# cts198859/deeprl_network

Measured on NVIDIA H100. Metric: agent-env-steps/sec CACC Catch-up NeurComm A2C, higher is better.
Workload: dtype f32

## Files before the change

### deeprl_network_b200/csrc/tc_wgrad.cu

```cuda
#include "bwd_common.cuh"
#include "tc_row.cuh"

extern long long* g_nmarl_prof;

namespace {
using namespace tcrow;

enum { J_GATE0 = 0, J_GATE1, J_ENC_X, J_ENC_M0, J_ENC_M1, J_COUNT };
constexpr int WG_LANES = 128, WG_HALF = 64;
constexpr int WG_A_THREADS = WG_LANES, WG_THREADS = WG_A_THREADS + 2 * 128;
constexpr uint32_t WG_A_TILE = WG_LANES * 128, WG_A_SLOT = 2 * WG_A_TILE;
constexpr uint32_t WG_RING = 224 * 1024;
constexpr int WG_MAX_BARS = 32;
constexpr size_t WG_SMEM = 1024 + WG_RING + WG_MAX_BARS * 8;
static_assert(WG_SMEM <= 232448, "wgrad rings exceed the 227 KB of dynamic shared memory");
static_assert(WG_HALF == ROWS, "each MMA warpgroup covers the 64 rows of one wgmma");
constexpr int WG_REGS_A = 120, WG_REGS_MMA = 192;
static_assert(WG_A_THREADS * WG_REGS_A + 256 * WG_REGS_MMA <= WG_THREADS * 168, "setmaxnreg split exceeds the CTA's registers");
constexpr int SEG_KB = 20;

__device__ __forceinline__ void wg_depths(int N, int& S, int& A) {
  S = N >= 256 ? 2 : (N >= 192 ? 3 : (N >= 128 ? 4 : 6));
  A = (int)((WG_RING - (uint32_t)S * 256u * (uint32_t)N) / WG_A_SLOT);
  if (A > 4) A = 4;
}

struct RingPos {
  int idx = 0; uint32_t ph = 0;
  __device__ __forceinline__ void next(int n) { if (++idx == n) { idx = 0; ph ^= 1u; } }
};

struct TcWgK {
  int B, T, splits, ndp;
  const float* sv_sh; const float* sv_xin; const float* dzT; const float* dpT;
  const float* h_seq; const float* done_pre;
  float* ws;
  long long ws_off[J_COUNT];
  int jobs[J_COUNT]; int n_jobs;
  int* err;
  long long* prof;
};

struct JobDesc {
  const float* A; int F_A, a_feat0, ka_cnt, ones;
  int p_feat0, p_cnt;
  const float* BT; int tile_rows, n_row0, N;
};

__device__ __forceinline__ JobDesc job_desc(const nmarl_model& m, const TcWgK& k, int kind, int i) {
  const nmarl_agent& ag = m.agent[i];
  JobDesc d;
  d.p_feat0 = 0; d.p_cnt = 0;
  const int SD = m.s_dim, LDI = m.kx_pad + m.kp_pad + m.km_pad;
  const int Km = (m.variant == NMARL_IC3) ? NH : ag.n_nbr * NH;
  if (kind == J_GATE0 || kind == J_GATE1) {
    const int mt = kind - J_GATE0;
    d.A = k.sv_sh; d.F_A = SD + NH; d.a_feat0 = 128 * mt; d.ka_cnt = max(0, min(128, SD + NH - 128 * mt)); d.ones = 0;
    d.BT = k.dzT; d.tile_rows = 256; d.n_row0 = 0; d.N = 256;
  } else if (kind == J_ENC_X) {
    d.A = k.sv_xin; d.F_A = LDI; d.a_feat0 = 0; d.ka_cnt = ag.x_nsrc * ag.x_w; d.ones = 1;
    if (m.variant == NMARL_NC) { d.p_feat0 = m.kx_pad; d.p_cnt = ag.n_nbr * m.n_a; }
    d.BT = k.dpT; d.tile_rows = k.ndp; d.n_row0 = 0; d.N = k.ndp;
  } else {
    const int mt = kind - J_ENC_M0;
    d.A = k.sv_xin; d.F_A = LDI; d.a_feat0 = m.kx_pad + m.kp_pad + 128 * mt; d.ka_cnt = max(0, min(128, Km - 128 * mt)); d.ones = 0;
    d.BT = k.dpT; d.tile_rows = k.ndp; d.n_row0 = (m.variant == NMARL_NC) ? 128 : 64; d.N = 64;
  }
  return d;
}

template <bool RAW>
__global__ void __launch_bounds__(WG_THREADS, 1) tc_wgrad_kernel(const __grid_constant__ nmarl_model m,
                                                                 const __grid_constant__ TcWgK k) {
  extern __shared__ uint8_t smem_raw[];
  uint8_t* smem = reinterpret_cast<uint8_t*>((reinterpret_cast<uintptr_t>(smem_raw) + 1023) & ~uintptr_t(1023));

  const int sp = blockIdx.x, jslot = blockIdx.y, i = blockIdx.z;
  const int kind = k.jobs[jslot];
  const JobDesc d = job_desc(m, k, kind, i);
  const int lanes = d.ka_cnt > 0 ? d.ka_cnt + d.ones + d.p_cnt : 0;
  const int nact = (lanes + WG_HALF - 1) / WG_HALF;
  if (nact == 0) return;
  int S, AS;
  wg_depths(d.N, S, AS);
  uint8_t* bst = smem;
  uint8_t* ast = smem + (size_t)S * 256 * d.N;
  uint64_t* bars = reinterpret_cast<uint64_t*>(smem + WG_RING);
  uint64_t *b_full = bars, *b_split = b_full + S, *b_empty = b_split + S, *a_full = b_empty + S, *a_empty = a_full + AS;

  const int N_agents = m.n_agent;
  const int tid = threadIdx.x, warp = tid >> 5;
  const int bpt = k.B / 32;
  const int kb_total = k.T * bpt;
  const int per = (kb_total + k.splits - 1) / k.splits;
  const int kb0 = sp * per, kb1 = min(kb_total, kb0 + per);
  const int nkb = (d.ka_cnt > 0) ? max(0, kb1 - kb0) : 0;
  float* wsj = k.ws + k.ws_off[jslot] + ((size_t)sp * N_agents + i) * 128 * d.N;

  if (tid == 0) {
    for (int s = 0; s < S; ++s) { tc::mbar_init(&b_full[s], 1); tc::mbar_init(&b_split[s], WG_A_THREADS); tc::mbar_init(&b_empty[s], 4 * nact); }
    for (int s = 0; s < AS; ++s) { tc::mbar_init(&a_full[s], WG_A_THREADS); tc::mbar_init(&a_empty[s], 4 * nact); }
    tc::fence_barrier_init();
  }
  __syncthreads();
  const uint32_t tile_bytes = (uint32_t)d.N * 128u;

  if (warp < WG_A_THREADS / 32) {
    asm volatile("setmaxnreg.dec.sync.aligned.u32 %0;" ::"n"(WG_REGS_A));
    const int row = tid;
    const bool on = row < WG_HALF * nact;
    const int ka = row;
    const bool one = d.ones && ka == d.ka_cnt;
    const bool is_p = ka > d.ka_cnt && ka <= d.ka_cnt + d.p_cnt;
    const bool real = on && (ka < d.ka_cnt || is_p);
    const int feat = is_p ? d.p_feat0 + (ka - d.ka_cnt - 1) : d.a_feat0 + ka;
    int hs_agent = -1, hs_unit = 0;
    bool hs_mask = false;
    if (k.h_seq != nullptr && real && !is_p) {
      if ((kind == J_GATE0 || kind == J_GATE1) && feat >= m.s_dim) { hs_agent = i; hs_unit = feat - m.s_dim; hs_mask = true; }
      else if ((kind == J_ENC_M0 || kind == J_ENC_M1) && m.variant == NMARL_NC) {
        const int fm = feat - (m.kx_pad + m.kp_pad);
        hs_agent = m.agent[i].nbr[fm / NH]; hs_unit = fm % NH;
      }
    }
    auto load_x = [&](int q, float (&x)[32]) {
      const int kb = kb0 + q, t = kb / bpt, rb = kb - t * bpt;
      if (hs_agent >= 0) {
        const float* src = k.h_seq + (((size_t)t * N_agents + hs_agent) * NH + hs_unit) * k.B + rb * 32;
#pragma unroll
        for (int p = 0; p < 8; ++p) {
          const float4 v = __ldg(reinterpret_cast<const float4*>(src + 4 * p));
          x[4 * p] = v.x; x[4 * p + 1] = v.y; x[4 * p + 2] = v.z; x[4 * p + 3] = v.w;
        }
        if (hs_mask) {
          const float* dn = k.done_pre + (size_t)t * k.B + rb * 32;
#pragma unroll
          for (int p = 0; p < 8; ++p) {
            const float4 v = __ldg(reinterpret_cast<const float4*>(dn + 4 * p));
            x[4 * p] *= 1.0f - v.x; x[4 * p + 1] *= 1.0f - v.y; x[4 * p + 2] *= 1.0f - v.z; x[4 * p + 3] *= 1.0f - v.w;
          }
        }
      } else if (real) {
        const float* src = d.A + (((size_t)t * N_agents + i) * d.F_A + feat) * k.B + rb * 32;
#pragma unroll
        for (int p = 0; p < 8; ++p) {
          const float4 v = __ldcs(reinterpret_cast<const float4*>(src + 4 * p));
          x[4 * p] = v.x; x[4 * p + 1] = v.y; x[4 * p + 2] = v.z; x[4 * p + 3] = v.w;
        }
      } else {
#pragma unroll
        for (int j = 0; j < 32; ++j) x[j] = one ? 1.0f : 0.0f;
      }
    };
    float xa[32], xb[32];
    RingPos as, bs;
    auto emit_a = [&](int q, float (&x)[32]) {
      tc::mbar_wait(&a_empty[as.idx], as.ph ^ 1, k.err, 11);
      if (on) {
        uint8_t* hi = ast + (size_t)as.idx * WG_A_SLOT;
#pragma unroll
        for (int c = 0; c < 4; ++c) {
          float x8[8];
#pragma unroll
          for (int j = 0; j < 8; ++j) x8[j] = x[8 * c + j];
          tc::st_hilo8(hi, hi + WG_A_TILE, (uint32_t)row, (uint32_t)(8 * c), x8);
        }
        tc::fence_proxy_async();
      }
      tc::mbar_arrive(&a_full[as.idx]);
      as.next(AS);
      if (q + 2 < nkb) load_x(q + 2, x);
      if constexpr (RAW) {
        tc::mbar_wait(&b_full[bs.idx], bs.ph, k.err, 31);
        float4* bhi = reinterpret_cast<float4*>(bst + (size_t)bs.idx * 2 * tile_bytes);
        float4* blo = reinterpret_cast<float4*>(bst + (size_t)bs.idx * 2 * tile_bytes + tile_bytes);
        for (uint32_t e = (uint32_t)tid; e < tile_bytes / 16; e += WG_A_THREADS) {
          const float4 v = bhi[e];
          float4 h, lo4;
          tc::split_tf32(v.x, h.x, lo4.x); tc::split_tf32(v.y, h.y, lo4.y);
          tc::split_tf32(v.z, h.z, lo4.z); tc::split_tf32(v.w, h.w, lo4.w);
          bhi[e] = h;
          blo[e] = lo4;
        }
        tc::fence_proxy_async();
        tc::mbar_arrive(&b_split[bs.idx]);
        bs.next(S);
      }
    };
    if (nkb > 0) load_x(0, xa);
    if (nkb > 1) load_x(1, xb);
    for (int q = 0; q < nkb; q += 2) {
      emit_a(q, xa);
      if (q + 1 < nkb) emit_a(q + 1, xb);
    }
  } else {
    const int g = warp / 4 - 1;
    if (g >= nact) return;
    asm volatile("setmaxnreg.inc.sync.aligned.u32 %0;" ::"n"(WG_REGS_MMA));
    const int t = tid - (g + 1) * 128, w = t >> 5, l = t & 31;
    const bool issuer = g == 0 && t == 0;
    float* out = wsj + g * WG_HALF + 16 * w + (l >> 2);
    long long* prof = (issuer && k.prof != nullptr && sp == 0 && i == 0) ? k.prof + (size_t)jslot * 1024 : nullptr;
    if (prof) { prof[0] = clock64(); prof[3] = kind | (d.N << 8); }
    auto fetch = [&](int q, int st) {
      const int kb = kb0 + q;
      const int tt = kb / bpt, rb = kb - tt * bpt;
      const size_t pair = (size_t)(2 * d.tile_rows * 128);
      const size_t off = RAW ? (size_t)tt * N_agents * bpt * pair + ((size_t)i * bpt + rb) * (pair / 2)
                             : (((size_t)tt * N_agents + i) * bpt + rb) * pair;
      const uint8_t* tile = reinterpret_cast<const uint8_t*>(d.BT) + off;
      uint8_t* dst = bst + (size_t)st * 2 * tile_bytes;
      tc::mbar_arrive_expect_tx(&b_full[st], RAW ? tile_bytes : 2 * tile_bytes);
      tc::bulk_g2s(dst, tile + (size_t)d.n_row0 * 128, tile_bytes, &b_full[st]);
      if (!RAW) tc::bulk_g2s(dst + tile_bytes, tile + (size_t)(d.tile_rows + d.n_row0) * 128, tile_bytes, &b_full[st]);
    };
    if (issuer)
      for (int q = 0; q < S && q < nkb; ++q) fetch(q, q);
    float acc[128];
#pragma unroll
    for (int j = 0; j < 128; ++j) acc[j] = 0.f;
    auto drain = [&](bool rmw) {
#pragma unroll
      for (int j = 0; j < 32; ++j) {
        if (8 * j < d.N) {
          const int n = 8 * j + 2 * (l & 3);
#pragma unroll
          for (int e = 0; e < 4; ++e) {
            float* o = out + (size_t)(n + (e & 1)) * 128 + 8 * (e >> 1);
            *o = rmw ? *o + acc[4 * j + e] : acc[4 * j + e];
          }
        }
      }
    };
    RingPos as, bs;
    for (int q = 0; q < nkb; ++q) {
      const bool seg_first = (q % SEG_KB) == 0;
      uint8_t* b = bst + (size_t)bs.idx * 2 * tile_bytes;
      if constexpr (RAW) tc::mbar_wait(&b_split[bs.idx], bs.ph, k.err, 33);
      else tc::mbar_wait(&b_full[bs.idx], bs.ph, k.err, 31);
      if (prof && q < 300) prof[4 + 3 * q] = clock64();
      tc::mbar_wait(&a_full[as.idx], as.ph, k.err, 32);
      if (prof && q < 300) prof[5 + 3 * q] = clock64();
      uint8_t* a = ast + (size_t)as.idx * WG_A_SLOT + g * (WG_A_TILE / 2);
      tc::wgmma_fence();
      tc::wgmma_kblock_3x(d.N, acc, tc::smem_desc_sw128(a), tc::smem_desc_sw128(a + WG_A_TILE), tc::smem_desc_sw128(b),
                          tc::smem_desc_sw128(b + tile_bytes), 4, seg_first);
      tc::wgmma_commit();
      tc::wgmma_wait_all();
      if (prof && q < 300) prof[6 + 3 * q] = clock64();
      if (l == 0) { tc::mbar_arrive(&a_empty[as.idx]); tc::mbar_arrive(&b_empty[bs.idx]); }
      if (issuer && q + S < nkb) {
        tc::mbar_wait(&b_empty[bs.idx], bs.ph, k.err, 34);
        fetch(q + S, bs.idx);
      }
      as.next(AS); bs.next(S);
      if ((q + 1) % SEG_KB == 0 || q + 1 == nkb) drain(q >= SEG_KB);
    }
    if (nkb == 0) drain(false);
    if (prof) { prof[1] = min(nkb, 300); prof[2] = clock64(); }
  }
}

__global__ void __launch_bounds__(256) tc_wgrad_reduce_kernel(const __grid_constant__ nmarl_model m, const __grid_constant__ TcWgK k,
                                                             float* __restrict__ grads) {
  const int jslot = blockIdx.y, i = blockIdx.z, kind = k.jobs[jslot];
  const JobDesc d = job_desc(m, k, kind, i);
  const nmarl_agent& ag = m.agent[i];
  const int lanes = d.ka_cnt + (d.ones ? 1 : 0) + d.p_cnt;
  const int total = 128 * d.N;
  for (int e = blockIdx.x * blockDim.x + threadIdx.x; e < total; e += gridDim.x * blockDim.x) {
    const int ln = e & 127, n = e >> 7;
    if (ln >= lanes) continue;
    float s = 0.f;
    for (int sp = 0; sp < k.splits; ++sp) s += k.ws[k.ws_off[jslot] + (((size_t)sp * m.n_agent + i) * d.N + n) * 128 + ln];
    if (kind == J_GATE0 || kind == J_GATE1) grads[ag.o_wxh + (size_t)(128 * (kind - J_GATE0) + ln) * NG + n] = s;
    else if (kind == J_ENC_X) {
      if (ln < d.ka_cnt) { if (n < NH) grads[ag.o_w_ob + ln * NH + n] = s; }
      else if (ln > d.ka_cnt) { if (n >= NH && n < 2 * NH) grads[ag.o_w_fp + (ln - d.ka_cnt - 1) * NH + n - NH] = s; }
      else if (n < NH) grads[ag.o_b_ob + n] = s;
      else if (m.variant == NMARL_NC && n < 2 * NH) grads[ag.o_b_fp + n - NH] = s;
      else if (ag.o_b_msg >= 0) grads[ag.o_b_msg + n - ((m.variant == NMARL_NC) ? 2 * NH : NH)] = s;
    } else grads[ag.o_w_msg + (size_t)(128 * (kind - J_ENC_M0) + ln) * NH + n] = s;
  }
}

__global__ void __launch_bounds__(256) gate_bias_reduce_kernel(const __grid_constant__ nmarl_model m, const float* __restrict__ part,
                                                              int tiles, int T, float* __restrict__ grads) {
  __shared__ float red[8][32];
  const int c = threadIdx.x & 31, p = threadIdx.x >> 5, col = blockIdx.x * 32 + c, i = blockIdx.y;
  const int n = T * tiles;
  float s = 0.f;
  for (int e = p; e < n; e += 8) {
    const int t = e / tiles, tile = e - t * tiles;
    s += part[(((size_t)t * m.n_agent + i) * tiles + tile) * NG + col];
  }
  red[p][c] = s;
  __syncthreads();
  if (p == 0) {
    float tsum = 0.f;
    for (int w = 0; w < 8; ++w) tsum += red[w][c];
    grads[m.agent[i].o_b + col] = tsum;
  }
}

NMARL_PARAMS_FIT(nmarl_model, TcWgK);
NMARL_PARAMS_FIT(nmarl_model, TcWgK, float*);
NMARL_PARAMS_FIT(nmarl_model, const float*, int, int, float*);

int job_list(const nmarl_model* m, int* jobs) {
  int n = 0;
  jobs[n++] = J_GATE0;
  if (m->s_dim + NH > 128) jobs[n++] = J_GATE1;
  jobs[n++] = J_ENC_X;
  if (m->variant != NMARL_IA2C) {
    jobs[n++] = J_ENC_M0;
    if (m->km_pad > 128) jobs[n++] = J_ENC_M1;
  }
  return n;
}
int job_N(const nmarl_model* m, int kind) {
  if (kind == J_GATE0 || kind == J_GATE1) return 256;
  if (kind == J_ENC_X) return nmarl_tc_ndp(m);
  return 64;
}

}

int nmarl_tc_ndp(const nmarl_model* m) { return m->variant == NMARL_NC ? 192 : (m->variant == NMARL_IA2C ? 64 : 128); }

int nmarl_tc_wgrad_splits(int n_agent) {
  int s = 33;
  while (4 * s * n_agent > 132 * 8 && s > 1) s = (s + 1) / 2;
  return s;
}

int64_t nmarl_tc_wgrad_ws_floats(const nmarl_model* m) {
  int jobs[J_COUNT];
  const int nj = job_list(m, jobs);
  int64_t tot = 0;
  for (int j = 0; j < nj; ++j) tot += (int64_t)nmarl_tc_wgrad_splits(m->n_agent) * m->n_agent * 128 * job_N(m, jobs[j]);
  return tot;
}

int nmarl_tc_launch_wgrads(const nmarl_model* m, int B, int T, const float* sv_sh, const float* sv_xin, const float* dzT,
                           const float* dpT, const float* sv_dz, float* ws, float* grads, int* err, cudaStream_t st,
                           cudaStream_t st_bias, bool raw_tiles, void** ev_wgrad, const float* h_seq, const float* done_pre) {
  TcWgK k{};
  k.B = B; k.T = T; k.splits = nmarl_tc_wgrad_splits(m->n_agent); k.ndp = nmarl_tc_ndp(m);
  k.sv_sh = sv_sh; k.sv_xin = sv_xin; k.dzT = dzT; k.dpT = dpT; k.ws = ws; k.err = err;
  k.h_seq = h_seq; k.done_pre = done_pre; k.prof = g_nmarl_prof;
  k.n_jobs = job_list(m, k.jobs);
  long long off = 0;
  for (int j = 0; j < k.n_jobs; ++j) { k.ws_off[j] = off; off += (long long)k.splits * m->n_agent * 128 * job_N(m, k.jobs[j]); }
  static bool configured = false;
  if (!configured) {
    NMARL_CUDA(cudaFuncSetAttribute(tc_wgrad_kernel<false>, cudaFuncAttributeMaxDynamicSharedMemorySize, (int)WG_SMEM));
    NMARL_CUDA(cudaFuncSetAttribute(tc_wgrad_kernel<true>, cudaFuncAttributeMaxDynamicSharedMemorySize, (int)WG_SMEM));
    configured = true;
  }
  gate_bias_reduce_kernel<<<dim3(NG / 32, m->n_agent), 256, 0, st_bias>>>(*m, sv_dz, B / 32, T, grads);
  NMARL_LAUNCH_CHECK();
  if (ev_wgrad) NMARL_CUDA(cudaEventRecord((cudaEvent_t)ev_wgrad[0], st));
  const dim3 grid(k.splits, k.n_jobs, m->n_agent);
  if (raw_tiles) tc_wgrad_kernel<true><<<grid, WG_THREADS, WG_SMEM, st>>>(*m, k);
  else tc_wgrad_kernel<false><<<grid, WG_THREADS, WG_SMEM, st>>>(*m, k);
  NMARL_LAUNCH_CHECK();
  if (ev_wgrad) NMARL_CUDA(cudaEventRecord((cudaEvent_t)ev_wgrad[1], st));
  NMARL_DBG_SYNC(st, "tc_wgrad_kernel");
  tc_wgrad_reduce_kernel<<<dim3(64, k.n_jobs, m->n_agent), 256, 0, st>>>(*m, k, grads);
  NMARL_LAUNCH_CHECK();
  NMARL_DBG_SYNC(st, "tc_wgrad_reduce");
  return 0;
}
```

Before: 52.82 million.

## Template wgrad MMA loop on N and keep one wgmma group in flight

The MMA warpgroups' main loop moves into a function templated on the tile width N, so the accumulator array and drain loops are sized at compile time instead of a fixed 128-register array with runtime guards. Each k-block's wgmma now waits only on the previous group (wait<1>), overlapping the next block's issue with the current one's completion before releasing ring slots and prefetching. The RAW-mode TF32 hi/lo split loop is also unrolled by four to batch shared-memory loads. In exchange the kernel holds more code per N instantiation, and an unsupported N now reports an error.

```diff
diff --git a/deeprl_network_b200/csrc/tc_wgrad.cu b/deeprl_network_b200/csrc/tc_wgrad.cu
--- a/deeprl_network_b200/csrc/tc_wgrad.cu
+++ b/deeprl_network_b200/csrc/tc_wgrad.cu
@@ -19,10 +19,10 @@
 static_assert(WG_A_THREADS * WG_REGS_A + 256 * WG_REGS_MMA <= WG_THREADS * 168, "setmaxnreg split exceeds the CTA's registers");
 constexpr int SEG_KB = 20;
 
-__device__ __forceinline__ void wg_depths(int N, int& S, int& A) {
-  S = N >= 256 ? 2 : (N >= 192 ? 3 : (N >= 128 ? 4 : 6));
-  A = (int)((WG_RING - (uint32_t)S * 256u * (uint32_t)N) / WG_A_SLOT);
-  if (A > 4) A = 4;
+__host__ __device__ constexpr int wg_stages(int N) { return N >= 256 ? 2 : (N >= 192 ? 3 : (N >= 128 ? 4 : 6)); }
+__host__ __device__ constexpr int wg_slots(int N) {
+  return (WG_RING - (uint32_t)wg_stages(N) * 256u * (uint32_t)N) / WG_A_SLOT >= 4
+             ? 4 : (int)((WG_RING - (uint32_t)wg_stages(N) * 256u * (uint32_t)N) / WG_A_SLOT);
 }
 
 struct RingPos {
@@ -69,6 +69,67 @@
   return d;
 }
 
+struct MmaRing {
+  uint8_t* bst; uint8_t* ast;
+  uint64_t *b_ready; int b_code;
+  uint64_t *b_empty, *a_full, *a_empty;
+  int* err;
+};
+
+template <int N, class Fetch>
+__device__ __forceinline__ void mma_job(const MmaRing& r, int nkb, bool issuer, int l, float* out, long long* prof,
+                                        const Fetch& fetch) {
+  constexpr int S = wg_stages(N), AS = wg_slots(N);
+  constexpr uint32_t TB = (uint32_t)N * 128u;
+  float acc[N / 2];
+#pragma unroll
+  for (int j = 0; j < N / 2; ++j) acc[j] = 0.f;
+  auto drain = [&](bool rmw) {
+#pragma unroll
+    for (int j = 0; j < N / 8; ++j) {
+      const int n = 8 * j + 2 * (l & 3);
+#pragma unroll
+      for (int e = 0; e < 4; ++e) {
+        float* o = out + (size_t)(n + (e & 1)) * 128 + 8 * (e >> 1);
+        *o = rmw ? *o + acc[4 * j + e] : acc[4 * j + e];
+      }
+    }
+  };
+  RingPos as, bs, rb;
+  int ra = 0;
+  auto release = [&](int q) {
+    if (prof && q < 300) prof[6 + 3 * q] = clock64();
+    if (l == 0) { tc::mbar_arrive(&r.a_empty[ra]); tc::mbar_arrive(&r.b_empty[rb.idx]); }
+    if (issuer && q + S < nkb) {
+      tc::mbar_wait(&r.b_empty[rb.idx], rb.ph, r.err, 34);
+      fetch(q + S, rb.idx);
+    }
+    ra = ra + 1 == AS ? 0 : ra + 1;
+    rb.next(S);
+  };
+  for (int q0 = 0; q0 < nkb; q0 += SEG_KB) {
+    const int q1 = min(nkb, q0 + SEG_KB);
+    for (int q = q0; q < q1; ++q) {
+      tc::mbar_wait(&r.b_ready[bs.idx], bs.ph, r.err, r.b_code);
+      if (prof && q < 300) prof[4 + 3 * q] = clock64();
+      tc::mbar_wait(&r.a_full[as.idx], as.ph, r.err, 32);
+      if (prof && q < 300) prof[5 + 3 * q] = clock64();
+      const uint8_t* a = r.ast + (size_t)as.idx * WG_A_SLOT;
+      const uint8_t* b = r.bst + (size_t)bs.idx * 2 * TB;
+      tc::wgmma_fence();
+      tc::wgmma_kblock_3x<N, 4>(acc, tc::smem_desc_sw128(a), tc::smem_desc_sw128(a + WG_A_TILE), tc::smem_desc_sw128(b),
+                                tc::smem_desc_sw128(b + TB), q == q0);
+      tc::wgmma_commit();
+      as.next(AS); bs.next(S);
+      if (q > q0) { tc::wgmma_wait<1>(); release(q - 1); }
+    }
+    tc::wgmma_wait<0>();
+    release(q1 - 1);
+    drain(q0 > 0);
+  }
+  if (nkb == 0) drain(false);
+}
+
 template <bool RAW>
 __global__ void __launch_bounds__(WG_THREADS, 1) tc_wgrad_kernel(const __grid_constant__ nmarl_model m,
                                                                  const __grid_constant__ TcWgK k) {
@@ -81,8 +142,7 @@
   const int lanes = d.ka_cnt > 0 ? d.ka_cnt + d.ones + d.p_cnt : 0;
   const int nact = (lanes + WG_HALF - 1) / WG_HALF;
   if (nact == 0) return;
-  int S, AS;
-  wg_depths(d.N, S, AS);
+  const int S = wg_stages(d.N), AS = wg_slots(d.N);
   uint8_t* bst = smem;
   uint8_t* ast = smem + (size_t)S * 256 * d.N;
   uint64_t* bars = reinterpret_cast<uint64_t*>(smem + WG_RING);
@@ -174,13 +234,18 @@
         tc::mbar_wait(&b_full[bs.idx], bs.ph, k.err, 31);
         float4* bhi = reinterpret_cast<float4*>(bst + (size_t)bs.idx * 2 * tile_bytes);
         float4* blo = reinterpret_cast<float4*>(bst + (size_t)bs.idx * 2 * tile_bytes + tile_bytes);
-        for (uint32_t e = (uint32_t)tid; e < tile_bytes / 16; e += WG_A_THREADS) {
-          const float4 v = bhi[e];
-          float4 h, lo4;
-          tc::split_tf32(v.x, h.x, lo4.x); tc::split_tf32(v.y, h.y, lo4.y);
-          tc::split_tf32(v.z, h.z, lo4.z); tc::split_tf32(v.w, h.w, lo4.w);
-          bhi[e] = h;
-          blo[e] = lo4;
+        for (uint32_t e0 = (uint32_t)tid; e0 < tile_bytes / 16; e0 += 4 * WG_A_THREADS) {
+          float4 v[4];
+#pragma unroll
+          for (int u = 0; u < 4; ++u) v[u] = bhi[e0 + u * WG_A_THREADS];
+#pragma unroll
+          for (int u = 0; u < 4; ++u) {
+            float4 h, lo4;
+            tc::split_tf32(v[u].x, h.x, lo4.x); tc::split_tf32(v[u].y, h.y, lo4.y);
+            tc::split_tf32(v[u].z, h.z, lo4.z); tc::split_tf32(v[u].w, h.w, lo4.w);
+            bhi[e0 + u * WG_A_THREADS] = h;
+            blo[e0 + u * WG_A_THREADS] = lo4;
+          }
         }
         tc::fence_proxy_async();
         tc::mbar_arrive(&b_split[bs.idx]);
@@ -216,47 +281,14 @@
     };
     if (issuer)
       for (int q = 0; q < S && q < nkb; ++q) fetch(q, q);
-    float acc[128];
-#pragma unroll
-    for (int j = 0; j < 128; ++j) acc[j] = 0.f;
-    auto drain = [&](bool rmw) {
-#pragma unroll
-      for (int j = 0; j < 32; ++j) {
-        if (8 * j < d.N) {
-          const int n = 8 * j + 2 * (l & 3);
-#pragma unroll
-          for (int e = 0; e < 4; ++e) {
-            float* o = out + (size_t)(n + (e & 1)) * 128 + 8 * (e >> 1);
-            *o = rmw ? *o + acc[4 * j + e] : acc[4 * j + e];
-          }
-        }
-      }
-    };
-    RingPos as, bs;
-    for (int q = 0; q < nkb; ++q) {
-      const bool seg_first = (q % SEG_KB) == 0;
-      uint8_t* b = bst + (size_t)bs.idx * 2 * tile_bytes;
-      if constexpr (RAW) tc::mbar_wait(&b_split[bs.idx], bs.ph, k.err, 33);
-      else tc::mbar_wait(&b_full[bs.idx], bs.ph, k.err, 31);
-      if (prof && q < 300) prof[4 + 3 * q] = clock64();
-      tc::mbar_wait(&a_full[as.idx], as.ph, k.err, 32);
-      if (prof && q < 300) prof[5 + 3 * q] = clock64();
-      uint8_t* a = ast + (size_t)as.idx * WG_A_SLOT + g * (WG_A_TILE / 2);
-      tc::wgmma_fence();
-      tc::wgmma_kblock_3x(d.N, acc, tc::smem_desc_sw128(a), tc::smem_desc_sw128(a + WG_A_TILE), tc::smem_desc_sw128(b),
-                          tc::smem_desc_sw128(b + tile_bytes), 4, seg_first);
-      tc::wgmma_commit();
-      tc::wgmma_wait_all();
-      if (prof && q < 300) prof[6 + 3 * q] = clock64();
-      if (l == 0) { tc::mbar_arrive(&a_empty[as.idx]); tc::mbar_arrive(&b_empty[bs.idx]); }
-      if (issuer && q + S < nkb) {
-        tc::mbar_wait(&b_empty[bs.idx], bs.ph, k.err, 34);
-        fetch(q + S, bs.idx);
-      }
-      as.next(AS); bs.next(S);
-      if ((q + 1) % SEG_KB == 0 || q + 1 == nkb) drain(q >= SEG_KB);
-    }
-    if (nkb == 0) drain(false);
+    const MmaRing r{bst, ast + g * (WG_A_TILE / 2), RAW ? b_split : b_full, RAW ? 33 : 31, b_empty, a_full, a_empty, k.err};
+    switch (d.N) {
+      case 64: mma_job<64>(r, nkb, issuer, l, out, prof, fetch); break;
+      case 128: mma_job<128>(r, nkb, issuer, l, out, prof, fetch); break;
+      case 192: mma_job<192>(r, nkb, issuer, l, out, prof, fetch); break;
+      case 256: mma_job<256>(r, nkb, issuer, l, out, prof, fetch); break;
+      default: atomicCAS(k.err, 0, 30); return;
+    }
     if (prof) { prof[1] = min(nkb, 300); prof[2] = clock64(); }
   }
 }
```

Result: no change. 53.22 million (median of 6 runs) (+0.8%).
